# modal-labs/modal-client

Hardware: AMD Instinct MI355X
Metric: map_items_per_sec (higher is better)
Workload: dtype bf16; 1 GPU; model=Function.map fan-out (BASELINE config 3), global_batch=12500, seq_len=0, parallelism=map1, dynamic_batching=64, chunk_items=256, workers=8

## Files before the change

csrc/core.cpp:

```cpp

#include <pybind11/pybind11.h>
#include <pybind11/stl.h>

#include "lane.h"
#include "ring.h"

#include <algorithm>
#include <atomic>
#include <functional>
#include <thread>
#include <cerrno>
#include <cstdint>
#include <cstring>
#include <fcntl.h>
#include <stdexcept>
#include <string>
#include <sys/mman.h>
#include <sys/stat.h>
#include <unistd.h>
#include <vector>

namespace py = pybind11;

namespace {

using modal_amd::BellFile;
using modal_amd::Ring;
using modal_amd::RingHub;

constexpr uint64_t kGilReleaseBytes = 64 * 1024;

bool ring_push(Ring& ring, py::buffer buf) {
  py::buffer_info info = buf.request();
  const uint8_t* src = static_cast<const uint8_t*>(info.ptr);
  const uint64_t n = (uint64_t)info.size * (uint64_t)info.itemsize;
  uint8_t* dst = ring.reserve(n);
  if (!dst) return false;
  if (n >= kGilReleaseBytes) {
    py::gil_scoped_release release;
    std::memcpy(dst, src, n);
  } else {
    std::memcpy(dst, src, n);
  }
  ring.commit();
  return true;
}

py::list ring_pop_all(Ring& ring, size_t max_frames) {
  py::list out;
  ring.pop(
      [&](const uint8_t* ptr, size_t len) {
        out.append(py::bytes(reinterpret_cast<const char*>(ptr), len));
      },
      max_frames);
  return out;
}

py::list hub_drain(RingHub& hub) {
  py::list out;
  hub.drain([&](int slot, const uint8_t* ptr, size_t len) {
    out.append(py::make_tuple(slot, py::bytes(reinterpret_cast<const char*>(ptr), len)));
  });
  return out;
}

using modal_amd::Assignment;
using modal_amd::ChunkDone;
using modal_amd::ChunkLane;
using modal_amd::FrameKind;

py::str sv_str(std::string_view s) { return py::str(s.data(), s.size()); }

py::tuple done_tuple(const ChunkDone& d) {
  py::object cis = py::none();
  if (!d.cis_nil) {
    py::list items;
    for (int64_t v : d.cis) items.append(py::int_(v));
    cis = std::move(items);
  }
  return py::make_tuple(sv_str(d.token), sv_str(d.call_id), sv_str(d.chunk_id),
                        sv_str(d.function_id), py::int_(d.count),
                        py::bytes(d.data.data(), d.data.size()), cis);
}

py::list assignment_list(const std::vector<Assignment>& assignments) {
  py::list out;
  for (const auto& a : assignments) out.append(py::make_tuple(a.token, a.worker_slot));
  return out;
}

py::object parse_chunk_done_py(py::buffer buf) {
  py::buffer_info info = buf.request();
  ChunkDone done;
  FrameKind kind = modal_amd::parse_chunk_done(
      static_cast<const uint8_t*>(info.ptr), (size_t)info.size * (size_t)info.itemsize, &done);
  if (kind != FrameKind::kDoneClean) return py::none();
  return done_tuple(done);
}

int lane_submit(ChunkLane& lane, int fn_slot, const std::string& token, uint64_t count,
                py::buffer frame, bool front) {
  py::buffer_info info = frame.request();
  return lane.submit(fn_slot, token, count, static_cast<const uint8_t*>(info.ptr),
                     (size_t)info.size * (size_t)info.itemsize, front);
}

py::tuple lane_drain(ChunkLane& lane, RingHub& hub) {
  py::list completions, raw;
  std::vector<Assignment> assignments;
  lane.drain(
      hub,
      [&](int slot, const ChunkDone& done) {
        completions.append(py::make_tuple(slot, done_tuple(done)));
      },
      [&](int slot, const uint8_t* ptr, size_t len) {
        raw.append(py::make_tuple(slot, py::bytes(reinterpret_cast<const char*>(ptr), len)));
      },
      &assignments);
  return py::make_tuple(completions, raw, assignment_list(assignments));
}

py::bytes pack_payloads(const std::vector<py::bytes>& items) {
  uint64_t total = 0;
  std::vector<std::pair<const char*, size_t>> views;
  views.reserve(items.size());
  for (const auto& item : items) {
    char* ptr;
    Py_ssize_t n;
    if (PyBytes_AsStringAndSize(item.ptr(), &ptr, &n) != 0)
      throw std::runtime_error("pack_payloads: not bytes");
// ... 319 lines not shown
  }
  if (pid < 0) {
    if (cg_fd >= 0) ::close(cg_fd);
    throw std::runtime_error("clone3: " + std::string(strerror(errno)));
  }
  if (pid == 0) {
    ::setsid();
    if (stdin_fd >= 0) ::dup2(stdin_fd, 0);
    if (stdout_fd >= 0) ::dup2(stdout_fd, 1);
    if (stderr_fd >= 0) ::dup2(stderr_fd, 2);
    for (int fd = 3; fd < 1024; ++fd) ::close(fd);
    if (!cwd.empty() && ::chdir(cwd.c_str()) != 0) _exit(126);
    if (rlimit_as_mib > 0) {
      struct rlimit rl;
      rl.rlim_cur = rl.rlim_max = (rlim_t)rlimit_as_mib << 20;
      ::setrlimit(RLIMIT_AS, &rl);
    }
    ::execve(cargv[0], cargv.data(), cenv.data());
    _exit(127);
  }
  if (cg_fd >= 0) ::close(cg_fd);
  return (int64_t)pid;
}


PYBIND11_MODULE(_core, m) {
  m.doc() = "modal_amd native core: shm ring transport + batch framing";
  py::class_<BellFile, std::shared_ptr<BellFile>>(m, "BellFile")
      .def(py::init<const std::string&, bool>(), py::arg("path"), py::arg("create") = false);
  py::class_<Ring, std::shared_ptr<Ring>>(m, "ShmRing")
      .def(py::init<const std::string&, uint64_t, bool>(), py::arg("path"),
           py::arg("capacity") = (uint64_t)64 << 20, py::arg("create") = false)
      .def("push", &ring_push)
      .def("pop_all", &ring_pop_all, py::arg("max_frames") = 0)
      .def("pending_bytes", &Ring::pending_bytes)
      .def("capacity", &Ring::capacity)
      .def("too_large", &Ring::too_large)
      .def("bell_wakes", &Ring::bell_wakes)
      .def("set_shared_bell", &Ring::set_shared_bell);
  py::class_<RingHub>(m, "RingHub")
      .def(py::init<const std::string&, int>(), py::arg("bell_path") = "",
           py::arg("timeout_ms") = 20)
      .def("add_ring", &RingHub::add_ring)
      .def("remove_ring", &RingHub::remove_ring)
      .def("fd", &RingHub::fd)
      .def("drain", &hub_drain)
      .def("close", &RingHub::close)
      .def("stats", [](RingHub& hub) {
        py::dict d;
        d["notifies"] = hub.notifies();
        d["waits"] = hub.waits();
        d["drains"] = hub.drains();
        d["producer_wakes"] = hub.producer_wakes();
        d["rings"] = hub.ring_count();
        return d;
      });
  py::class_<ChunkLane>(m, "ChunkLane")
      .def(py::init<>())
      .def("add_worker", &ChunkLane::add_worker)
      .def("remove_worker", &ChunkLane::remove_worker)
      .def("set_eligible", &ChunkLane::set_eligible)
      .def("set_cap", &ChunkLane::set_cap, py::arg("fn_slot"), py::arg("items"),
           py::arg("min_chunks") = 1)
      .def("submit", &lane_submit, py::arg("fn_slot"), py::arg("token"), py::arg("count"),
           py::arg("frame"), py::arg("front") = false)
      .def("kick", [](ChunkLane& lane, int fn_slot) {
        std::vector<Assignment> out;
        lane.kick(fn_slot, &out);
        return assignment_list(out);
      })
      .def("complete", [](ChunkLane& lane, int worker_slot, const std::string& token) {
        std::vector<Assignment> out;
        lane.complete(worker_slot, token, &out);
        return assignment_list(out);
      })
      .def("cancel", &ChunkLane::cancel)
      .def("drop_queue", &ChunkLane::drop_queue)
      .def("drain", &lane_drain)
      .def("queued", &ChunkLane::queued)
      .def("inflight", &ChunkLane::inflight)
      .def("outstanding_items", &ChunkLane::outstanding_items)
      .def("pushed", &ChunkLane::pushed);
  m.def("parse_chunk_done", &parse_chunk_done_py);
  m.def("pack_payloads", &pack_payloads);
  m.def("malz_compress", &malz_compress, py::arg("data"), py::arg("min_gain") = 0.95);
  m.def("malz_decompress", &malz_decompress);
  m.def("unpack_payloads", &unpack_payloads);
  m.def("spawn_supervised", &spawn_supervised, py::arg("argv"), py::arg("cwd"),
        py::arg("env"), py::arg("cgroup_dir") = "", py::arg("rlimit_as_mib") = 0,
        py::arg("stdin_fd") = -1, py::arg("stdout_fd") = -1, py::arg("stderr_fd") = -1,
        "clone3(CLONE_INTO_CGROUP) + execve supervisor (atomic cgroup placement)");
}
```

csrc/lane.h:

```cpp

#pragma once

#include <algorithm>
#include <cstdint>
#include <cstring>
#include <deque>
#include <memory>
#include <string>
#include <string_view>
#include <unordered_map>
#include <unordered_set>
#include <utility>
#include <vector>

#include "ring.h"

namespace modal_amd {


struct MsgReader {
  const uint8_t* p;
  const uint8_t* end;

  bool need(size_t n) const { return (size_t)(end - p) >= n; }
// ... 198 lines not shown
        if (r.need(1) && *r.p == 0xc0) {
          r.p++;
          out->cis_nil = true;
          break;
        }
        uint64_t n;
        ok = r.read_array_header(&n) && n <= (uint64_t)(r.end - r.p);
        out->cis_nil = false;
        out->cis.clear();
        for (uint64_t k = 0; ok && k < n; k++) {
          int64_t v;
          ok = r.read_int(&v);
          if (ok) out->cis.push_back(v);
        }
        break;
      }
    }
    if (!ok) {
      r.p = value_at;
      if (!r.skip()) return FrameKind::kOther;
      clean = false;
      if (bit == T) return FrameKind::kOther;
      if (bit == TOKEN) has_token = false;
    }
  }
  if (r.p != r.end) return FrameKind::kOther;
  if (!is_done || !has_token) return FrameKind::kOther;
  out->token = token;
  if (clean && seen == 255) return FrameKind::kDoneClean;
  return FrameKind::kDoneOther;
}


struct Assignment {
  std::string token;
  int worker_slot;
};

class ChunkLane {
 public:
  void add_worker(int slot, std::shared_ptr<Ring> ring) {
    Worker& w = workers_[slot];
    w.ring = std::move(ring);
  }

  std::vector<std::string> remove_worker(int slot) {
    std::vector<std::string> tokens;
    auto it = workers_.find(slot);
    if (it == workers_.end()) return tokens;
    for (auto& entry : it->second.inflight) tokens.push_back(entry.first);
    workers_.erase(it);
    for (auto& fn : fns_) fn.second.eligible.erase(slot);
    return tokens;
  }

  void set_eligible(int fn_slot, int worker_slot, bool on) {
    Fn& fn = fns_[fn_slot];
    if (on && workers_.count(worker_slot)) fn.eligible.insert(worker_slot);
    else fn.eligible.erase(worker_slot);
  }

  void set_cap(int fn_slot, uint64_t items, uint32_t min_chunks) {
    Fn& fn = fns_[fn_slot];
    fn.cap_items = items;
    fn.min_chunks = min_chunks;
  }
// ... 6 lines not shown
      if (slot >= 0) return slot;
    }
    Queued q{token, count, std::string(reinterpret_cast<const char*>(frame), len)};
    if (front) fn.queue.push_front(std::move(q));
    else fn.queue.push_back(std::move(q));
    return -1;
  }

  void kick(int fn_slot, std::vector<Assignment>* out) {
    auto it = fns_.find(fn_slot);
    if (it == fns_.end()) return;
    Fn& fn = it->second;
    while (!fn.queue.empty()) {
      Queued& q = fn.queue.front();
      int slot = place(fn_slot, fn, q.token, q.count,
                       reinterpret_cast<const uint8_t*>(q.frame.data()), q.frame.size(),
                       fn.queue.size());
      if (slot < 0) break;
      out->push_back(Assignment{std::move(q.token), slot});
      fn.queue.pop_front();
    }
  }

  bool complete(int worker_slot, std::string_view token, std::vector<Assignment>* out) {
    auto wit = workers_.find(worker_slot);
    if (wit == workers_.end()) return false;
    Worker& w = wit->second;
    auto it = w.inflight.find(std::string(token));
    if (it == w.inflight.end()) return false;
    int fn_slot = it->second.fn_slot;
    Load& load = w.load[fn_slot];
    load.items -= std::min(load.items, it->second.count);
    if (load.chunks) load.chunks--;
    w.inflight.erase(it);
    kick(fn_slot, out);
    return true;
  }

  std::vector<std::string> cancel(const std::vector<std::string>& tokens) {
    std::unordered_set<std::string_view> drop(tokens.begin(), tokens.end());
    std::vector<std::string> dropped;
    for (auto& entry : fns_) {
      auto& q = entry.second.queue;
      auto keep = q.begin();
      for (auto it = q.begin(); it != q.end(); ++it) {
        if (drop.count(it->token)) {
          dropped.push_back(std::move(it->token));
        } else {
          if (keep != it) *keep = std::move(*it);
          ++keep;
        }
      }
      q.erase(keep, q.end());
    }
    return dropped;
  }

  std::vector<std::string> drop_queue(int fn_slot) {
    std::vector<std::string> tokens;
    auto it = fns_.find(fn_slot);
    if (it == fns_.end()) return tokens;
    for (auto& q : it->second.queue) tokens.push_back(std::move(q.token));
    it->second.queue.clear();
    return tokens;
  }

  template <typename OnClean, typename OnRaw>
  void drain(RingHub& hub, OnClean&& on_clean, OnRaw&& on_raw, std::vector<Assignment>* out) {
    ChunkDone done;
    hub.drain([&](int slot, const uint8_t* ptr, size_t len) {
      FrameKind kind = parse_chunk_done(ptr, len, &done);
      if (kind != FrameKind::kOther) complete(slot, done.token, out);
      if (kind == FrameKind::kDoneClean) on_clean(slot, done);
      else on_raw(slot, ptr, len);
    });
  }

  size_t queued(int fn_slot) const {
    auto it = fns_.find(fn_slot);
    return it == fns_.end() ? 0 : it->second.queue.size();
  }

  size_t inflight(int worker_slot) const {
    auto it = workers_.find(worker_slot);
    return it == workers_.end() ? 0 : it->second.inflight.size();
  }

  uint64_t outstanding_items(int fn_slot, int worker_slot) const {
    auto it = workers_.find(worker_slot);
    if (it == workers_.end()) return 0;
    auto lit = it->second.load.find(fn_slot);
    return lit == it->second.load.end() ? 0 : lit->second.items;
  }

  uint64_t pushed() const { return pushed_; }

 private:
  struct Queued {
    std::string token;
    uint64_t count;
    std::string frame;
  };
  struct Load {
    uint64_t items = 0;
    uint32_t chunks = 0;
  };
  struct Inflight {
    int fn_slot;
    uint64_t count;
  };
  struct Worker {
    std::shared_ptr<Ring> ring;
    std::unordered_map<int, Load> load;
    std::unordered_map<std::string, Inflight> inflight;
  };
  struct Fn {
    uint64_t cap_items = 256;
    uint32_t min_chunks = 1;
    std::deque<Queued> queue;
    std::unordered_set<int> eligible;
  };

  static bool has_credit(const Fn& fn, const Load& load, size_t backlog) {
    if (load.items < fn.cap_items) return true;
    return load.chunks < fn.min_chunks && backlog > fn.eligible.size();
  }

  int place(int fn_slot, Fn& fn, const std::string& token, uint64_t count,
            const uint8_t* frame, size_t len, size_t backlog) {
    std::vector<std::pair<uint64_t, int>> order;
    for (int slot : fn.eligible) {
      auto it = workers_.find(slot);
      if (it == workers_.end()) continue;
      const Load& load = it->second.load[fn_slot];
      if (has_credit(fn, load, backlog)) order.emplace_back(load.items, slot);
    }
    std::sort(order.begin(), order.end());
    for (auto& cand : order) {
      Worker& w = workers_[cand.second];
      if (w.ring->too_large(len) || !w.ring->push(frame, len)) continue;
      Load& load = w.load[fn_slot];
      load.items += count;
      load.chunks++;
      w.inflight[token] = Inflight{fn_slot, count};
      pushed_++;
      return cand.second;
    }
    return -1;
  }

  std::unordered_map<int, Worker> workers_;
  std::unordered_map<int, Fn> fns_;
  uint64_t pushed_ = 0;
};

}
```

csrc/ring.h:

```cpp

#pragma once

#include <atomic>
#include <cerrno>
#include <climits>
#include <cstdint>
#include <cstring>
#include <ctime>
#include <fcntl.h>
#include <linux/futex.h>
#include <memory>
#include <csignal>
#include <pthread.h>
#include <mutex>
#include <stdexcept>
#include <string>
#include <sys/eventfd.h>
#include <sys/mman.h>
#include <sys/stat.h>
#include <sys/syscall.h>
#include <thread>
#include <unistd.h>
#include <utility>
#include <vector>
// ... 92 lines not shown
      ::close(fd_);
      throw std::runtime_error("ShmRing: mmap failed");
    }
    base_ = static_cast<uint8_t*>(mem);
    header_ = reinterpret_cast<RingHeader*>(base_);
    data_ = base_ + sizeof(RingHeader);
    total_ = total;
    if (create) {
      header_->head.store(0, std::memory_order_relaxed);
      header_->tail.store(0, std::memory_order_relaxed);
      header_->capacity = capacity;
      header_->bell.seq.store(0, std::memory_order_relaxed);
      header_->bell.waiting.store(0, std::memory_order_relaxed);
      header_->bell.wakes.store(0, std::memory_order_relaxed);
      header_->magic = kMagic;
    } else if (header_->magic != kMagic || header_->capacity != capacity) {
      ::munmap(base_, total_);
      ::close(fd_);
      throw std::runtime_error("ShmRing: magic mismatch");
    }
    capacity_ = capacity;
  }

  ~Ring() {
    if (base_) ::munmap(base_, total_);
    if (fd_ >= 0) ::close(fd_);
  }

  Ring(const Ring&) = delete;
  Ring& operator=(const Ring&) = delete;

  bool too_large(uint64_t n) const { return n + 8 > capacity_ || n >= kSkip; }

  uint8_t* reserve(uint64_t n) {
    if (too_large(n)) throw std::runtime_error("frame larger than ring");
    uint64_t head = header_->head.load(std::memory_order_relaxed);
    uint64_t tail = header_->tail.load(std::memory_order_acquire);
    uint64_t pos = head % capacity_;
    uint64_t to_end = capacity_ - pos;
    uint64_t need = 4 + n;
    uint64_t skip = to_end < need ? to_end : 0;
    if (head + skip + need - tail > capacity_) return nullptr;
    if (skip) {
      if (to_end >= 4) {
        uint32_t sentinel = kSkip;
        std::memcpy(data_ + pos, &sentinel, 4);
      }
      pos = 0;
    }
    uint32_t len32 = (uint32_t)n;
    std::memcpy(data_ + pos, &len32, 4);
    pending_commit_ = head + skip + need;
    return data_ + pos + 4;
  }

  void commit() {
    header_->head.store(pending_commit_, std::memory_order_release);
    bell_ring(header_->bell);
    if (shared_bell_) bell_ring(*shared_bell_->bell());
  }

  bool push(const uint8_t* src, uint64_t n) {
    uint8_t* dst = reserve(n);
    if (!dst) return false;
    std::memcpy(dst, src, n);
    commit();
    return true;
  }

  template <typename F>
  size_t pop(F&& cb, size_t max_frames = 0) {
    uint64_t tail = header_->tail.load(std::memory_order_relaxed);
    uint64_t head = header_->head.load(std::memory_order_acquire);
    if (tail == head) return 0;
    size_t count = 0;
    while (tail < head) {
      uint64_t pos = tail % capacity_;
      uint64_t to_end = capacity_ - pos;
      if (to_end < 4) {
        tail += to_end;
        continue;
      }
      uint32_t len32;
      std::memcpy(&len32, data_ + pos, 4);
      if (len32 == kSkip) {
        tail += to_end;
        continue;
      }
      if ((uint64_t)len32 + 4 > to_end || tail + 4 + len32 > head) break;
      cb(static_cast<const uint8_t*>(data_ + pos + 4), (size_t)len32);
      tail += 4 + len32;
      if (max_frames && ++count >= max_frames) break;
    }
    header_->tail.store(tail, std::memory_order_release);
    return count;
  }

  bool has_pending() const {
    return header_->head.load(std::memory_order_acquire) !=
           header_->tail.load(std::memory_order_acquire);
  }

  uint64_t pending_bytes() const {
    return header_->head.load(std::memory_order_acquire) -
           header_->tail.load(std::memory_order_acquire);
  }

  uint64_t capacity() const { return capacity_; }
  Bell* bell() const { return &header_->bell; }
  uint32_t bell_wakes() const { return header_->bell.wakes.load(std::memory_order_relaxed); }

  void set_shared_bell(std::shared_ptr<BellFile> bell) { shared_bell_ = std::move(bell); }

 private:
  int fd_ = -1;
  uint8_t* base_ = nullptr;
  uint8_t* data_ = nullptr;
  RingHeader* header_ = nullptr;
  uint64_t capacity_ = 0;
  uint64_t total_ = 0;
  uint64_t pending_commit_ = 0;
  std::shared_ptr<BellFile> shared_bell_;
};

class RingHub {
 public:
  explicit RingHub(const std::string& bell_path = "", int timeout_ms = 20)
      : timeout_ms_(timeout_ms < 1 ? 1 : timeout_ms) {
    if (!bell_path.empty()) {
      bell_file_ = std::make_shared<BellFile>(bell_path, true);
      bell_ = bell_file_->bell();
    }
    efd_ = ::eventfd(0, EFD_NONBLOCK | EFD_CLOEXEC);
    if (efd_ < 0) throw std::runtime_error("RingHub: eventfd failed");
    thread_ = std::thread([this] { run(); });
  }

  ~RingHub() { close(); }
  RingHub(const RingHub&) = delete;
  RingHub& operator=(const RingHub&) = delete;

  void add_ring(int slot, std::shared_ptr<Ring> ring) {
    std::lock_guard<std::mutex> lock(mu_);
    for (auto& entry : rings_) {
      if (entry.first == slot) {
        entry.second = std::move(ring);
        return;
      }
    }
    if (!bell_) {
      bell_owner_ = ring;
      bell_ = ring->bell();
    }
    rings_.emplace_back(slot, std::move(ring));
// ... 119 lines not shown
```

modal_amd/runtime/worker.py:

```python

from __future__ import annotations

import asyncio
import contextvars
import inspect
import os
import sys
import time
import traceback
from concurrent.futures import ThreadPoolExecutor
from typing import Any, Optional

from .._serialization import (
    DataFormat,
    GeneratorDone,
    deserialize,
    deserialize_payload,
    serialize,
    serialize_data_format,
    set_client_context,
)
from ..scheduler.blobs import INLINE_LIMIT, BlobStore
from ..scheduler.calls import (
    GENERIC_STATUS_FAILURE,
    GENERIC_STATUS_INTERNAL_FAILURE,
    GENERIC_STATUS_SUCCESS,
    GENERIC_STATUS_TERMINATED,
    GENERIC_STATUS_TIMEOUT,
)
from ..exception import InputCancellation
from ..scheduler.transport import Connection
from .execution_context import _reset_current_context, _set_current_context

HEARTBEAT_INTERVAL = 15.0
OUTPUT_FLUSH_INTERVAL = 0.001
OUTPUT_BATCH_MAX = 512

_app_id_var: contextvars.ContextVar[str] = contextvars.ContextVar("modal_amd_app_id", default="")

import threading as _threading

_slot_tls = _threading.local()


def _slot_streams_enabled() -> bool:
    torch = sys.modules.get("torch")
    cuda = getattr(torch, "cuda", None) if torch is not None else None
    try:
        return (
            cuda is not None
            and os.environ.get("MODAL_AMD_SLOT_STREAMS", "0") not in ("0", "false")
            and cuda.is_initialized()
        )
    except AttributeError:
        return False


def _invoke_on_slot_stream(fn: Any, args: tuple, kwargs: dict) -> Any:
    torch = sys.modules.get("torch")
    cuda = getattr(torch, "cuda", None) if torch is not None else None
    try:
        if (
            cuda is None
            or os.environ.get("MODAL_AMD_SLOT_STREAMS", "0") in ("0", "false")
            or not cuda.is_initialized()
        ):
            return fn(*args, **kwargs)
    except AttributeError:
        return fn(*args, **kwargs)
    stream = getattr(_slot_tls, "stream", None)
    if stream is None:
        stream = torch.cuda.Stream()
        _slot_tls.stream = stream
    with torch.cuda.stream(stream):
        result = fn(*args, **kwargs)
# ... 707 lines not shown
            prefix = f"in-{call_id[3:]}-"
            plain_call = not _slot_streams_enabled()
            tok_c = _current_function_call_id.set(call_id)
            tok_a = _app_id_var.set(frt.app_id)
            self._register_sync_thread(msg["token"])
            try:
                for ci in range(start, end):
                    tok_i = _current_input_id.set(prefix + str(ci))
                    try:
                        if kw_common is None:
                            args, kwargs = pairs[ci]
                        else:
                            args, kwargs = pairs[ci], kw_common
                        if plain_call:
                            values[ci] = fn(*args, **kwargs)
                        else:
                            values[ci] = _invoke_on_slot_stream(fn, args, kwargs)
                    except InputCancellation:
                        raise
                    except BaseException as exc:
                        errors[ci] = (
                            self._serialize_exception(exc),
                            "".join(traceback.format_exception_only(type(exc), exc)).strip(),
                        )
                    finally:
                        _current_input_id.reset(tok_i)
            finally:
                self._unregister_sync_thread(msg["token"])
                _current_function_call_id.reset(tok_c)
                _app_id_var.reset(tok_a)

        from .execution_context import _current_function_call_id, _current_input_id

        try:
            fn0 = await loop.run_in_executor(self.executor, frt.load)
            if frt._service is not None:
                fn0 = frt.get_callable(msg.get("method", ""))
        except BaseException as exc:
            data = self._serialize_exception(exc)
            err = "".join(traceback.format_exception_only(type(exc), exc)).strip()
            for ci in range(count):
                errors[ci] = (data, err)
            fn0 = None

        app_tok = _app_id_var.set(frt.app_id)
        try:
            if fn0 is not None and frt.batch_max_size > 1:
                is_async = inspect.iscoroutinefunction(fn0)

                def _transpose(pairs: Any, kw_common: Any, idxs: range) -> tuple:
                    rows = [
                        (pairs[ci], kw_common) if kw_common is not None else pairs[ci]
                        for ci in idxs
                    ]
                    if kw_common is not None:
                        n_args = len(rows[0][0]) if rows else 0
                        arglists = [[row[0][i] for row in rows] for i in range(n_args)]
                        kwlists = {k: [v] * len(rows) for k, v in kw_common.items()}
                    else:
                        n_args = max((len(a) for a, _ in rows), default=0)
                        arglists = [
                            [a[i] if i < len(a) else None for a, _ in rows]
                            for i in range(n_args)
                        ]
                        keys: set = set()
                        for _, kw in rows:
                            keys.update(kw)
                        kwlists = {k: [kw.get(k) for _, kw in rows] for k in keys}
                    return tuple(arglists), kwlists

                def _store(idxs: range, results: Any) -> None:
                    if not isinstance(results, (list, tuple)) or len(results) != len(idxs):
                        raise ValueError(
                            f"Batched function {frt.name} must return a list of "
                            f"{len(idxs)} results, got {type(results).__name__}"
                        )
                    for ci, r in zip(idxs, results):
                        values[ci] = r

                try:
                    pairs, kw_common = await loop.run_in_executor(
                        self.executor, self._chunk_pairs, msg["chunk_id"]
                    )
                    bsz = frt.batch_max_size
                    async with frt.sem:
                        for start in range(0, count, bsz):
                            idxs = range(start, min(start + bsz, count))
                            try:
                                arglists, kwlists = _transpose(pairs, kw_common, idxs)
                                if is_async:
                                    results = await self._execute(frt, fn0, arglists, kwlists)
                                else:

                                    def _call_batch(
                                        arglists: tuple = arglists, kwlists: dict = kwlists
                                    ) -> Any:
                                        tok_c = _current_function_call_id.set(call_id)
                                        tok_a2 = _app_id_var.set(frt.app_id)
                                        try:
                                            return fn0(*arglists, **kwlists)
                                        finally:
                                            _current_function_call_id.reset(tok_c)
                                            _app_id_var.reset(tok_a2)

                                    results = await loop.run_in_executor(
                                        self.executor, _call_batch
                                    )
                                _store(idxs, results)
                            except (asyncio.CancelledError, InputCancellation):
                                raise
                            except BaseException as exc:
                                data = self._serialize_exception(exc)
                                err = "".join(
                                    traceback.format_exception_only(type(exc), exc)
                                ).strip()
                                for ci in idxs:
                                    errors[ci] = (data, err)
                except (asyncio.CancelledError, InputCancellation):
                    raise
                except BaseException as exc:
                    data = self._serialize_exception(exc)
                    err = "".join(traceback.format_exception_only(type(exc), exc)).strip()
                    for ci in range(count):
                        errors.setdefault(ci, (data, err))
            elif fn0 is not None and (
                inspect.iscoroutinefunction(fn0) or inspect.isasyncgenfunction(fn0)
            ):
                item = {"chunk": msg["chunk_id"], "ci": 0}
                for ci in range(count):
                    item["ci"] = ci
                    try:
                        args, kwargs = await loop.run_in_executor(
                            self.executor, self._resolve_item_args, dict(item)
                        )
                        values[ci] = await self._execute(frt, fn0, args, kwargs)
                    except BaseException as exc:
                        errors[ci] = (
                            self._serialize_exception(exc),
                            "".join(traceback.format_exception_only(type(exc), exc)).strip(),
                        )
            elif fn0 is not None:
                if count <= frt.max_concurrent:
                    n_ranges = count
                else:
                    n_ranges = min(frt.max_concurrent, max(1, count // 16))
                size = (count + n_ranges - 1) // n_ranges

                async def run_one(start: int, end: int) -> None:
                    async with frt.sem:
                        await loop.run_in_executor(self.executor, run_range, start, end)

                await asyncio.gather(
                    *(run_one(s, min(s + size, count)) for s in range(0, count, size))
                )
        except (asyncio.CancelledError, InputCancellation):
            return
        finally:
            _app_id_var.reset(app_tok)

        reply: dict[str, Any] = {
            "t": "chunk_done",
            "token": token,
            "call_id": call_id,
            "chunk_id": msg["chunk_id"],
            "function_id": frt.function_id,
            "count": count,
        }
        if errors:
            reply["exceptions"] = {str(ci): [d, r] for ci, (d, r) in errors.items()}
        if values:
            ordered_cis = sorted(values)
            from ._serialize_chunk import serialize_value_chunk

            def pack() -> tuple:
                return serialize_value_chunk([values[ci] for ci in ordered_cis])

            data, per_item = await loop.run_in_executor(self.executor, pack)
            if data is not None:
                reply["data"] = data
                reply["cis"] = None if len(ordered_cis) == count else ordered_cis
            else:
                reply["items"] = {str(ci): b for ci, b in zip(ordered_cis, per_item)}
        try:
            await self.conn.send(reply)
        except Exception:
            pass

    async def _run_frame_fast(self, frt: FunctionRuntime, items: list[dict]) -> None:
        loop = asyncio.get_running_loop()
        from .execution_context import _current_function_call_id, _current_input_id

        def run_all() -> Any:
            results: list[dict] = []
            try:
                fn = frt.get_callable(items[0].get("method", ""))
            except BaseException as exc:
                err = "".join(traceback.format_exception_only(type(exc), exc)).strip()
                data = self._serialize_exception(exc)
                return [
                    self._make_output(
                        item["token"], frt.function_id, GENERIC_STATUS_FAILURE, data,
                        DataFormat.PICKLE, err,
                    )
                    for item in items
                ]
            if inspect.iscoroutinefunction(fn) or inspect.isasyncgenfunction(fn) or inspect.isgeneratorfunction(fn):
                return None
            values: list = []
            value_tokens: list[str] = []
            for item in items:
                if item["token"] in self._abandoned:
                    self._abandoned.discard(item["token"])
                    continue
                call_id = item["token"].rsplit(":", 2)[0]
                tok_i = _current_input_id.set(item.get("input_id"))
                tok_c = _current_function_call_id.set(call_id)
                try:
                    args, kwargs = self._resolve_item_args(item)
                    values.append(fn(*args, **kwargs))
# ... 335 lines not shown
```

modal_amd/scheduler/transport.py:

```python

from __future__ import annotations

import asyncio
import os
import itertools
import struct
from collections import deque
from typing import Any, Awaitable, Callable, Optional

import msgpack

_LEN = struct.Struct("<I")

MAX_FRAME = 1 << 31

RING_MIN_FRAME = int(os.environ.get("MODAL_AMD_RING_MIN", 32 * 1024))
RING_CAPACITY = 64 << 20

try:
    from .. import _core
except ImportError:
    _core = None


# ... 17 lines not shown
    except (asyncio.IncompleteReadError, ConnectionResetError):
        return None
    (length,) = _LEN.unpack(header)
    if length > MAX_FRAME:
        raise ValueError(f"Frame too large: {length}")
    try:
        body = await reader.readexactly(length)
    except (asyncio.IncompleteReadError, ConnectionResetError):
        return None
    return msgpack.unpackb(body, raw=False, strict_map_key=False)


class Connection:

    def __init__(
        self,
        reader: asyncio.StreamReader,
        writer: asyncio.StreamWriter,
        handler: Callable[[dict], Awaitable[None]],
        rpc_target: Optional[Any] = None,
    ):
        self.reader = reader
        self.writer = writer
        self.handler = handler
        self.rpc_target = rpc_target
        self._rpc_seq = itertools.count(1)
        self._pending: dict[int, asyncio.Future] = {}
        self._send_lock = asyncio.Lock()
        self._closed = asyncio.Event()
        self._reader_task: Optional[asyncio.Task] = None
        self._loop: Optional[asyncio.AbstractEventLoop] = None
        self.ring_out: Any = None
        self.ring_in: Any = None
        self.ring_frames_sent = 0
        self.ring_frames_received = 0
        self._lane = False
        self._own_hub: Any = None
        self.sync_handler: Optional[Callable[[dict], bool]] = None
        self._inbox: deque = deque()
        self._lane_waiting = 0
        self._inbox_task: Optional[asyncio.Task] = None

    def attach_rings(self, out_path: Optional[str], in_path: Optional[str], create: bool) -> bool:
        if _core is None or not out_path or not in_path:
            return False
        try:
            self.ring_out = _core.ShmRing(out_path, RING_CAPACITY, create)
            self.ring_in = _core.ShmRing(in_path, RING_CAPACITY, create)
            return True
        except Exception:
            self.ring_out = None
            self.ring_in = None
            return False

    def enable_lane(self, shared_bell: Optional[str] = None, own_hub: bool = False) -> bool:
        if _core is None or self.ring_out is None or self.ring_in is None:
            return False
        try:
            if shared_bell:
                self.ring_out.set_shared_bell(_core.BellFile(shared_bell, False))
            if own_hub:
                hub = _core.RingHub("", 20)
                hub.add_ring(0, self.ring_in)
                asyncio.get_running_loop().add_reader(hub.fd(), self._on_own_hub_ready)
                self._own_hub = hub
        except Exception:
            self._drop_own_hub()
            return False
        self._lane = True
        return True

    def _on_own_hub_ready(self) -> None:
        hub = self._own_hub
        if hub is None:
# ... 12 lines not shown

    def on_ring_frame(self, body: bytes) -> None:
        self.ring_frames_received += 1
        msg = msgpack.unpackb(body, raw=False, strict_map_key=False)
        if self._inbox_task is None:
            if msg.get("t") in _RPC_REPLY_KINDS:
                self._on_rpc_reply(msg)
                return
            if self.sync_handler is not None and self.sync_handler(msg):
                return
            self._inbox_task = asyncio.get_running_loop().create_task(self._run_inbox())
        self._inbox.append(msg)

    async def _run_inbox(self) -> None:
        try:
            while self._inbox:
                msg = self._inbox.popleft()
                try:
                    await self._dispatch(msg)
                except asyncio.CancelledError:
                    raise
                except Exception:
                    pass
        finally:
            self._inbox_task = None
            if self._inbox and not self._closed.is_set():
                self._inbox_task = asyncio.get_running_loop().create_task(self._run_inbox())

    async def _send_lane(self, body: bytes) -> None:
        if self._closed.is_set():
            raise ConnectionError("connection closed")
        ring = self.ring_out
        if self._lane_waiting == 0 and ring.push(body):
            self.ring_frames_sent += 1
            return
        self._lane_waiting += 1
        try:
            async with self._send_lock:
                while not ring.push(body):
                    if self._closed.is_set():
                        raise ConnectionError("connection closed")
                    await asyncio.sleep(0.001)
                self.ring_frames_sent += 1
        finally:
            self._lane_waiting -= 1

    def start(self) -> None:
        self._loop = asyncio.get_running_loop()
        self._reader_task = self._loop.create_task(self._read_loop())

    @property
    def closed(self) -> bool:
        return self._closed.is_set()

    async def wait_closed(self) -> None:
        await self._closed.wait()

    async def send(self, msg: dict, via_socket: bool = False) -> None:
        body = msgpack.packb(msg, use_bin_type=True)
        if self._lane and not via_socket:
            await self._send_lane(body)
            return
        if self.ring_out is not None and len(body) >= RING_MIN_FRAME and not via_socket:
            pushed = self.ring_out.push(body)
            if pushed:
                self.ring_frames_sent += 1
                async with self._send_lock:
                    self.writer.write(pack({"t": "rb"}))
                    await self.writer.drain()
                return
        data = _LEN.pack(len(body)) + body
        async with self._send_lock:
            self.writer.write(data)
            await self.writer.drain()

    async def call(self, method: str, params: Any = None, timeout: Optional[float] = None) -> Any:
        running = asyncio.get_running_loop()
        if self._loop is not None and running is not self._loop:
            fut = asyncio.run_coroutine_threadsafe(self.call(method, params, timeout), self._loop)
            return await asyncio.wrap_future(fut)
        rpc_id = next(self._rpc_seq)
        fut: asyncio.Future = asyncio.get_running_loop().create_future()
        self._pending[rpc_id] = fut
        try:
            await self.send({"t": "rpc", "i": rpc_id, "m": method, "p": params})
            if timeout is not None:
                return await asyncio.wait_for(fut, timeout)
            return await fut
        finally:
            self._pending.pop(rpc_id, None)

    async def _dispatch(self, msg: dict) -> None:
        kind = msg.get("t")
        if kind == "rpc":
            asyncio.get_running_loop().create_task(self._serve_rpc(msg))
        elif kind in _RPC_REPLY_KINDS:
            self._on_rpc_reply(msg)
        else:
            await self.handler(msg)
# ... 82 lines not shown
```

modal_amd/scheduler/workerhost.py:

```python

from __future__ import annotations

import asyncio
import heapq
import os
import subprocess
import sys
import time
from collections import deque
from typing import TYPE_CHECKING, Any, Optional

import msgpack

from ..utils.ids import new_id
from .calls import (
    GENERIC_STATUS_INTERNAL_FAILURE,
    MAX_INTERNAL_FAILURE_COUNT,
    FunctionDef,
    InputRecord,
)
from .transport import Connection, _core, native_lane_enabled

_CPU_COUNT = os.cpu_count()

# ... 155 lines not shown
                "call_id": record.call_id,
                "chunk_id": group.chunk_id,
                "token": group.token,
                "count": group.count,
                "payload": chunk.get("data"),
                "method": group.method,
                "max_concurrent": fdef.max_concurrent_inputs,
            },
            use_bin_type=True,
        )
        if len(frame) > LANE_MAX_FRAME:
            return False
        fn_slot = self._lane_fn_slot(fdef)
        token = group.token
        self._lane_groups[token] = (record, group)
        slot = self._lane.submit(fn_slot, token, group.count, frame, front)
        if slot >= 0:
            self._lane_assigned(token, slot)
        else:
            self._lane_refresh_fns.add(fdef.function_id)
            self._dispatch_wake.set()
        return True

    def _lane_assigned(self, token: str, slot: int) -> None:
        entry = self._lane_groups.get(token)
        w = self._lane_workers.get(slot)
        if entry is None or w is None:
            return
        record, group = entry
        group.state = "inflight"
        group.worker_id = w.worker_id
        w.last_active = time.time()
        w.inflight[token] = ("g", record, group)
        w.conn.ring_frames_sent += 1
        fid = record.function_id
        w.outstanding[fid] = w.outstanding.get(fid, 0) + group.count

    def _lane_revoke(self, w: WorkerHandle) -> None:
        if self._lane is not None and w.hub_slot is not None:
            for fid in w.lane_fns:
                self._lane.set_eligible(self._lane_fn_slots[fid], w.hub_slot, False)
        w.lane_fns.clear()

    async def _lane_dispatch(self) -> None:
        lane = self._lane
        for fid in list(self._lane_refresh_fns):
            self._lane_refresh_fns.discard(fid)
            fn_slot = self._lane_fn_slots.get(fid)
            if lane is None or fn_slot is None:
                continue
            fdef = self.scheduler.functions.get(fid)
            if fdef is None:
                for token in lane.drop_queue(fn_slot):
                    self._lane_groups.pop(token, None)
                continue
            fn_slot = self._lane_fn_slot(fdef)
            await self.ensure_workers(fdef.needs_gpu)
            candidates = [
                w
                for w in self.workers.values()
                if w.alive and not w.draining and (w.has_gpu or not fdef.needs_gpu)
            ]
            candidates = self._apply_placement(fdef, candidates)
            chosen = {w.worker_id for w in candidates}
            for w in list(self._lane_workers.values()):
                if fid in w.lane_fns and w.worker_id not in chosen:
                    w.lane_fns.discard(fid)
# ... 876 lines not shown
```

Baseline: 1.707 million items/s.

## Run chunk jobs in one executor call and push chunk_done natively from the worker thread

Map-chunk execution on the worker becomes a single executor job that runs the function, serializes the results and encodes the chunk_done reply straight into the shared-memory ring in C++ with the GIL released. This removes event-loop round trips, Python msgpack packing and a copy per chunk. The ring gains a producer mutex so several threads can push safely, and its push counter now tracks frames sent. It also adds per-chunk turnaround timing (clock_gettime on placement and completion) and a stress test, which cost a little per chunk and add some complexity around cancellation.

```diff
diff --git a/csrc/core.cpp b/csrc/core.cpp
--- a/csrc/core.cpp
+++ b/csrc/core.cpp
@@ -34,16 +34,11 @@
   py::buffer_info info = buf.request();
   const uint8_t* src = static_cast<const uint8_t*>(info.ptr);
   const uint64_t n = (uint64_t)info.size * (uint64_t)info.itemsize;
-  uint8_t* dst = ring.reserve(n);
-  if (!dst) return false;
   if (n >= kGilReleaseBytes) {
     py::gil_scoped_release release;
-    std::memcpy(dst, src, n);
-  } else {
-    std::memcpy(dst, src, n);
-  }
-  ring.commit();
-  return true;
+    return ring.push(src, n);
+  }
+  return ring.push(src, n);
 }
 
 py::list ring_pop_all(Ring& ring, size_t max_frames) {
@@ -96,6 +91,65 @@
       static_cast<const uint8_t*>(info.ptr), (size_t)info.size * (size_t)info.itemsize, &done);
   if (kind != FrameKind::kDoneClean) return py::none();
   return done_tuple(done);
+}
+
+struct DoneFields {
+  std::string_view token, call_id, chunk_id, function_id, data;
+  uint64_t count;
+  size_t size;
+};
+
+std::string_view ascii_view(const py::str& s, const char* what) {
+  if (!PyUnicode_IS_ASCII(s.ptr()))
+    throw py::value_error(std::string("chunk_done: ") + what + " is not ASCII");
+  Py_ssize_t n = 0;
+  const char* ptr = PyUnicode_AsUTF8AndSize(s.ptr(), &n);
+  if (!ptr) throw py::error_already_set();
+  if ((uint64_t)n > 0xffffffffULL)
+    throw py::value_error(std::string("chunk_done: ") + what + " is too long");
+  return std::string_view(ptr, (size_t)n);
+}
+
+DoneFields done_fields(const py::str& token, const py::str& call_id, const py::str& chunk_id,
+                       const py::str& function_id, int64_t count,
+                       const py::buffer_info& data) {
+  if (count < 0) throw py::value_error("chunk_done: count is negative");
+  DoneFields f;
+  f.token = ascii_view(token, "token");
+  f.call_id = ascii_view(call_id, "call_id");
+  f.chunk_id = ascii_view(chunk_id, "chunk_id");
+  f.function_id = ascii_view(function_id, "function_id");
+  uint64_t n = (uint64_t)data.size * (uint64_t)data.itemsize;
+  if (n > 0xffffffffULL) throw py::value_error("chunk_done: data is too long");
+  f.data = std::string_view(static_cast<const char*>(data.ptr), (size_t)n);
+  f.count = (uint64_t)count;
+  f.size = modal_amd::chunk_done_size(f.token, f.call_id, f.chunk_id, f.function_id, f.count,
+                                      f.data.size());
+  return f;
+}
+
+py::bytes build_chunk_done(const py::str& token, const py::str& call_id,
+                           const py::str& chunk_id, const py::str& function_id,
+                           int64_t count, py::buffer data) {
+  py::buffer_info info = data.request();
+  DoneFields f = done_fields(token, call_id, chunk_id, function_id, count, info);
+  py::bytes out(nullptr, (ssize_t)f.size);
+  uint8_t* dst = reinterpret_cast<uint8_t*>(PyBytes_AsString(out.ptr()));
+  modal_amd::encode_chunk_done(dst, f.token, f.call_id, f.chunk_id, f.function_id, f.count,
+                               f.data);
+  return out;
+}
+
+bool ring_push_chunk_done(Ring& ring, const py::str& token, const py::str& call_id,
+                          const py::str& chunk_id, const py::str& function_id,
+                          int64_t count, py::buffer data) {
+  py::buffer_info info = data.request();
+  DoneFields f = done_fields(token, call_id, chunk_id, function_id, count, info);
+  py::gil_scoped_release release;
+  return ring.push_with(f.size, [&](uint8_t* dst) {
+    modal_amd::encode_chunk_done(dst, f.token, f.call_id, f.chunk_id, f.function_id, f.count,
+                                 f.data);
+  });
 }
 
 int lane_submit(ChunkLane& lane, int fn_slot, const std::string& token, uint64_t count,
@@ -481,6 +535,9 @@
       .def(py::init<const std::string&, uint64_t, bool>(), py::arg("path"),
            py::arg("capacity") = (uint64_t)64 << 20, py::arg("create") = false)
       .def("push", &ring_push)
+      .def("push_chunk_done", &ring_push_chunk_done, py::arg("token"), py::arg("call_id"),
+           py::arg("chunk_id"), py::arg("function_id"), py::arg("count"), py::arg("data"))
+      .def("pushed", &Ring::pushed)
       .def("pop_all", &ring_pop_all, py::arg("max_frames") = 0)
       .def("pending_bytes", &Ring::pending_bytes)
       .def("capacity", &Ring::capacity)
@@ -529,8 +586,18 @@
       .def("queued", &ChunkLane::queued)
       .def("inflight", &ChunkLane::inflight)
       .def("outstanding_items", &ChunkLane::outstanding_items)
-      .def("pushed", &ChunkLane::pushed);
+      .def("pushed", &ChunkLane::pushed)
+      .def("stats", [](ChunkLane& lane, int fn_slot, bool reset) {
+        ChunkLane::Turnaround t = lane.stats(fn_slot, reset);
+        py::dict d;
+        d["chunks"] = t.chunks;
+        d["sum_ns"] = t.sum_ns;
+        d["max_ns"] = t.max_ns;
+        return d;
+      }, py::arg("fn_slot"), py::arg("reset") = false);
   m.def("parse_chunk_done", &parse_chunk_done_py);
+  m.def("build_chunk_done", &build_chunk_done, py::arg("token"), py::arg("call_id"),
+        py::arg("chunk_id"), py::arg("function_id"), py::arg("count"), py::arg("data"));
   m.def("pack_payloads", &pack_payloads);
   m.def("malz_compress", &malz_compress, py::arg("data"), py::arg("min_gain") = 0.95);
   m.def("malz_decompress", &malz_decompress);
diff --git a/csrc/lane.h b/csrc/lane.h
--- a/csrc/lane.h
+++ b/csrc/lane.h
@@ -254,6 +254,87 @@
 }
 
 
+inline size_t mp_str_size(size_t n) {
+  return n + (n < 32 ? 1 : n < 256 ? 2 : n < 65536 ? 3 : 5);
+}
+inline size_t mp_bin_size(size_t n) { return n + (n < 256 ? 2 : n < 65536 ? 3 : 5); }
+inline size_t mp_uint_size(uint64_t v) {
+  return v < 128 ? 1 : v < 256 ? 2 : v < 65536 ? 3 : v <= 0xffffffffULL ? 5 : 9;
+}
+
+inline uint8_t* mp_put_be(uint8_t* p, uint64_t v, int n) {
+  for (int i = n - 1; i >= 0; i--) *p++ = (uint8_t)(v >> (8 * i));
+  return p;
+}
+inline uint8_t* mp_put_str(uint8_t* p, std::string_view s) {
+  size_t n = s.size();
+  if (n < 32) *p++ = (uint8_t)(0xa0 | n);
+  else if (n < 256) { *p++ = 0xd9; p = mp_put_be(p, n, 1); }
+  else if (n < 65536) { *p++ = 0xda; p = mp_put_be(p, n, 2); }
+  else { *p++ = 0xdb; p = mp_put_be(p, n, 4); }
+  if (n) std::memcpy(p, s.data(), n);
+  return p + n;
+}
+inline uint8_t* mp_put_bin(uint8_t* p, std::string_view s) {
+  size_t n = s.size();
+  if (n < 256) { *p++ = 0xc4; p = mp_put_be(p, n, 1); }
+  else if (n < 65536) { *p++ = 0xc5; p = mp_put_be(p, n, 2); }
+  else { *p++ = 0xc6; p = mp_put_be(p, n, 4); }
+  if (n) std::memcpy(p, s.data(), n);
+  return p + n;
+}
+inline uint8_t* mp_put_uint(uint8_t* p, uint64_t v) {
+  if (v < 128) { *p++ = (uint8_t)v; return p; }
+  if (v < 256) { *p++ = 0xcc; return mp_put_be(p, v, 1); }
+  if (v < 65536) { *p++ = 0xcd; return mp_put_be(p, v, 2); }
+  if (v <= 0xffffffffULL) { *p++ = 0xce; return mp_put_be(p, v, 4); }
+  *p++ = 0xcf;
+  return mp_put_be(p, v, 8);
+}
+
+constexpr size_t kChunkDoneFixed =
+    1 + 2 + 11 + 6 + 8 + 9 + 12 + 6 + 5 + 4 + 1;
+
+inline size_t chunk_done_size(std::string_view token, std::string_view call_id,
+                              std::string_view chunk_id, std::string_view function_id,
+                              uint64_t count, size_t data_len) {
+  return kChunkDoneFixed + mp_str_size(token.size()) + mp_str_size(call_id.size()) +
+         mp_str_size(chunk_id.size()) + mp_str_size(function_id.size()) +
+         mp_uint_size(count) + mp_bin_size(data_len);
+}
+
+inline uint8_t* encode_chunk_done(uint8_t* dst, std::string_view token,
+                                  std::string_view call_id, std::string_view chunk_id,
+                                  std::string_view function_id, uint64_t count,
+                                  std::string_view data) {
+  uint8_t* p = dst;
+  *p++ = 0x88;
+  p = mp_put_str(p, "t");
+  p = mp_put_str(p, "chunk_done");
+  p = mp_put_str(p, "token");
+  p = mp_put_str(p, token);
+  p = mp_put_str(p, "call_id");
+  p = mp_put_str(p, call_id);
+  p = mp_put_str(p, "chunk_id");
+  p = mp_put_str(p, chunk_id);
+  p = mp_put_str(p, "function_id");
+  p = mp_put_str(p, function_id);
+  p = mp_put_str(p, "count");
+  p = mp_put_uint(p, count);
+  p = mp_put_str(p, "data");
+  p = mp_put_bin(p, data);
+  p = mp_put_str(p, "cis");
+  *p++ = 0xc0;
+  return p;
+}
+
+
+inline uint64_t monotonic_ns() {
+  struct timespec ts;
+  ::clock_gettime(CLOCK_MONOTONIC, &ts);
+  return (uint64_t)ts.tv_sec * 1000000000ULL + (uint64_t)ts.tv_nsec;
+}
+
 struct Assignment {
   std::string token;
   int worker_slot;
@@ -326,6 +407,12 @@
     Load& load = w.load[fn_slot];
     load.items -= std::min(load.items, it->second.count);
     if (load.chunks) load.chunks--;
+    uint64_t now = monotonic_ns();
+    uint64_t took = now > it->second.placed_ns ? now - it->second.placed_ns : 0;
+    Turnaround& t = fns_[fn_slot].turnaround;
+    t.chunks++;
+    t.sum_ns += took;
+    t.max_ns = std::max(t.max_ns, took);
     w.inflight.erase(it);
     kick(fn_slot, out);
     return true;
@@ -389,6 +476,20 @@
 
   uint64_t pushed() const { return pushed_; }
 
+  struct Turnaround {
+    uint64_t chunks = 0;
+    uint64_t sum_ns = 0;
+    uint64_t max_ns = 0;
+  };
+
+  Turnaround stats(int fn_slot, bool reset = false) {
+    auto it = fns_.find(fn_slot);
+    if (it == fns_.end()) return Turnaround{};
+    Turnaround t = it->second.turnaround;
+    if (reset) it->second.turnaround = Turnaround{};
+    return t;
+  }
+
  private:
   struct Queued {
     std::string token;
@@ -402,6 +503,7 @@
   struct Inflight {
     int fn_slot;
     uint64_t count;
+    uint64_t placed_ns;
   };
   struct Worker {
     std::shared_ptr<Ring> ring;
@@ -413,6 +515,7 @@
     uint32_t min_chunks = 1;
     std::deque<Queued> queue;
     std::unordered_set<int> eligible;
+    Turnaround turnaround;
   };
 
   static bool has_credit(const Fn& fn, const Load& load, size_t backlog) {
@@ -436,7 +539,7 @@
       Load& load = w.load[fn_slot];
       load.items += count;
       load.chunks++;
-      w.inflight[token] = Inflight{fn_slot, count};
+      w.inflight[token] = Inflight{fn_slot, count, monotonic_ns()};
       pushed_++;
       return cand.second;
     }
diff --git a/csrc/ring.h b/csrc/ring.h
--- a/csrc/ring.h
+++ b/csrc/ring.h
@@ -148,6 +148,24 @@
 
   bool too_large(uint64_t n) const { return n + 8 > capacity_ || n >= kSkip; }
 
+  template <typename W>
+  bool push_with(uint64_t n, W&& writer) {
+    std::lock_guard<std::mutex> lock(producer_mu_);
+    uint8_t* dst = reserve(n);
+    if (!dst) return false;
+    writer(dst);
+    commit();
+    pushed_.fetch_add(1, std::memory_order_relaxed);
+    return true;
+  }
+
+  bool push(const uint8_t* src, uint64_t n) {
+    return push_with(n, [&](uint8_t* dst) { std::memcpy(dst, src, n); });
+  }
+
+  uint64_t pushed() const { return pushed_.load(std::memory_order_relaxed); }
+
+ private:
   uint8_t* reserve(uint64_t n) {
     if (too_large(n)) throw std::runtime_error("frame larger than ring");
     uint64_t head = header_->head.load(std::memory_order_relaxed);
@@ -176,14 +194,7 @@
     if (shared_bell_) bell_ring(*shared_bell_->bell());
   }
 
-  bool push(const uint8_t* src, uint64_t n) {
-    uint8_t* dst = reserve(n);
-    if (!dst) return false;
-    std::memcpy(dst, src, n);
-    commit();
-    return true;
-  }
-
+ public:
   template <typename F>
   size_t pop(F&& cb, size_t max_frames = 0) {
     uint64_t tail = header_->tail.load(std::memory_order_relaxed);
@@ -236,6 +247,8 @@
   uint64_t capacity_ = 0;
   uint64_t total_ = 0;
   uint64_t pending_commit_ = 0;
+  std::mutex producer_mu_;
+  std::atomic<uint64_t> pushed_{0};
   std::shared_ptr<BellFile> shared_bell_;
 };
 
diff --git a/csrc/ring_producers_stress.cpp b/csrc/ring_producers_stress.cpp
--- /dev/null
+++ b/csrc/ring_producers_stress.cpp
@@ -0,0 +1,139 @@
+
+#include <atomic>
+#include <cstdio>
+#include <cstdlib>
+#include <string>
+#include <thread>
+#include <vector>
+
+#include "lane.h"
+#include "ring.h"
+
+using namespace modal_amd;
+
+namespace {
+
+constexpr int kProducers = 3;
+constexpr int kFrames = 20000;
+constexpr uint64_t kRingBytes = 64 * 1024;
+constexpr size_t kPlainHeader = 10;
+
+#define CHECK(cond)                                                      \
+  do {                                                                   \
+    if (!(cond)) {                                                       \
+      std::fprintf(stderr, "CHECK failed: %s (line %d)\n", #cond, __LINE__); \
+      std::abort();                                                      \
+    }                                                                    \
+  } while (0)
+
+size_t body_len(int producer, int seq) {
+  return 1024 + (size_t)(((uint32_t)seq * 2654435761u + (uint32_t)producer * 40503u) % 3072);
+}
+
+void fill(uint8_t* dst, size_t n, int producer, int seq) {
+  uint32_t x = (uint32_t)seq * 747796405u + (uint32_t)producer + 1u;
+  for (size_t i = 0; i < n; i++) {
+    x = x * 1664525u + 1013904223u;
+    dst[i] = (uint8_t)(x >> 24);
+  }
+}
+
+uint32_t checksum(const uint8_t* p, size_t n) {
+  uint32_t h = 2166136261u;
+  for (size_t i = 0; i < n; i++) h = (h ^ p[i]) * 16777619u;
+  return h;
+}
+
+void produce(Ring& ring, int producer) {
+  std::vector<uint8_t> body;
+  for (int seq = 0; seq < kFrames; seq++) {
+    size_t n = body_len(producer, seq);
+    body.resize(n);
+    fill(body.data(), n, producer, seq);
+    uint32_t sum = checksum(body.data(), n);
+    if (seq % 4 == 3) {
+      std::string token = "p" + std::to_string(producer) + ":" + std::to_string(seq);
+      std::string_view data(reinterpret_cast<const char*>(body.data()), n);
+      size_t size = chunk_done_size(token, "fc-stress", token.substr(1), "fu-stress", sum, n);
+      auto write = [&](uint8_t* dst) {
+        uint8_t* end = encode_chunk_done(dst, token, "fc-stress", token.substr(1), "fu-stress",
+                                         sum, data);
+        CHECK((size_t)(end - dst) == size);
+      };
+      while (!ring.push_with(size, write)) std::this_thread::yield();
+    } else {
+      auto write = [&](uint8_t* dst) {
+        dst[0] = 'P';
+        dst[1] = (uint8_t)producer;
+        uint32_t seq32 = (uint32_t)seq;
+        std::memcpy(dst + 2, &seq32, 4);
+        std::memcpy(dst + 6, &sum, 4);
+        std::memcpy(dst + kPlainHeader, body.data(), n);
+      };
+      while (!ring.push_with(kPlainHeader + n, write)) std::this_thread::yield();
+    }
+  }
+}
+
+}
+
+int main() {
+  char dir_template[] = "/tmp/ring-producers-XXXXXX";
+  CHECK(::mkdtemp(dir_template) != nullptr);
+  std::string dir = dir_template;
+  {
+    Ring tx(dir + "/ring", kRingBytes, true);
+    Ring rx(dir + "/ring", 0, false);
+
+    std::vector<std::thread> producers;
+    for (int p = 0; p < kProducers; p++) producers.emplace_back([&tx, p] { produce(tx, p); });
+
+    std::vector<int> next_seq(kProducers, 0);
+    int total = 0, encoded = 0;
+    ChunkDone done;
+    while (total < kProducers * kFrames) {
+      size_t got = rx.pop([&](const uint8_t* ptr, size_t len) {
+        int producer, seq;
+        uint32_t sum;
+        const uint8_t* body;
+        size_t n;
+        CHECK(len > kPlainHeader);
+        if (ptr[0] == 'P') {
+          producer = ptr[1];
+          uint32_t seq32;
+          std::memcpy(&seq32, ptr + 2, 4);
+          std::memcpy(&sum, ptr + 6, 4);
+          seq = (int)seq32;
+          body = ptr + kPlainHeader;
+          n = len - kPlainHeader;
+        } else {
+          CHECK(parse_chunk_done(ptr, len, &done) == FrameKind::kDoneClean);
+          CHECK(done.cis_nil && done.call_id == "fc-stress" && done.function_id == "fu-stress");
+          CHECK(done.token.size() > 3 && done.token[0] == 'p' && done.token[2] == ':');
+          CHECK(done.chunk_id == done.token.substr(1));
+          producer = done.token[1] - '0';
+          seq = std::atoi(std::string(done.token.substr(3)).c_str());
+          sum = (uint32_t)done.count;
+          body = reinterpret_cast<const uint8_t*>(done.data.data());
+          n = done.data.size();
+          CHECK(seq % 4 == 3);
+          encoded++;
+        }
+        CHECK(producer >= 0 && producer < kProducers);
+        CHECK(seq == next_seq[producer]);
+        next_seq[producer]++;
+        CHECK(n == body_len(producer, seq));
+        CHECK(checksum(body, n) == sum);
+        total++;
+      });
+      if (!got) std::this_thread::yield();
+    }
+    for (auto& t : producers) t.join();
+    CHECK(!rx.has_pending());
+    CHECK(tx.pushed() == (uint64_t)kProducers * kFrames);
+    CHECK(encoded == kProducers * (kFrames / 4));
+    std::printf("ring_producers_stress ok: %d frames, %d encoded natively\n", total, encoded);
+  }
+  std::string cmd = "rm -rf " + dir;
+  return std::system(cmd.c_str()) == 0 ? 0 : 1;
+}
diff --git a/modal_amd/runtime/worker.py b/modal_amd/runtime/worker.py
--- a/modal_amd/runtime/worker.py
+++ b/modal_amd/runtime/worker.py
@@ -41,6 +41,22 @@
 import threading as _threading
 
 _slot_tls = _threading.local()
+
+
+def _chunk_job_enabled() -> bool:
+    return os.environ.get("MODAL_AMD_CHUNK_JOB", "1").lower() not in ("0", "false", "no")
+
+
+class _ChunkJob:
+
+    __slots__ = ("lock", "cancelled")
+
+    def __init__(self) -> None:
+        self.lock = _threading.Lock()
+        self.cancelled = False
+
+
+_JOB_CANCELLED = object()
 
 
 def _slot_streams_enabled() -> bool:
@@ -814,8 +830,13 @@
 
         from .execution_context import _current_function_call_id, _current_input_id
 
+        chunk_job = frt.batch_max_size > 1 and _chunk_job_enabled()
+        job_reply: Any = None
         try:
-            fn0 = await loop.run_in_executor(self.executor, frt.load)
+            if chunk_job and frt._loaded:
+                fn0 = frt.load()
+            else:
+                fn0 = await loop.run_in_executor(self.executor, frt.load)
             if frt._service is not None:
                 fn0 = frt.get_callable(msg.get("method", ""))
         except BaseException as exc:
@@ -860,51 +881,114 @@
                     for ci, r in zip(idxs, results):
                         values[ci] = r
 
-                try:
-                    pairs, kw_common = await loop.run_in_executor(
-                        self.executor, self._chunk_pairs, msg["chunk_id"]
-                    )
-                    bsz = frt.batch_max_size
-                    async with frt.sem:
-                        for start in range(0, count, bsz):
-                            idxs = range(start, min(start + bsz, count))
+                if chunk_job and not is_async:
+                    state = _ChunkJob()
+
+                    def _run_job() -> Any:
+                        tok_c = _current_function_call_id.set(call_id)
+                        tok_a2 = _app_id_var.set(frt.app_id)
+                        self._register_sync_thread(token)
+                        try:
                             try:
-                                arglists, kwlists = _transpose(pairs, kw_common, idxs)
-                                if is_async:
-                                    results = await self._execute(frt, fn0, arglists, kwlists)
-                                else:
-
-                                    def _call_batch(
-                                        arglists: tuple = arglists, kwlists: dict = kwlists
-                                    ) -> Any:
-                                        tok_c = _current_function_call_id.set(call_id)
-                                        tok_a2 = _app_id_var.set(frt.app_id)
-                                        try:
-                                            return fn0(*arglists, **kwlists)
-                                        finally:
-                                            _current_function_call_id.reset(tok_c)
-                                            _app_id_var.reset(tok_a2)
-
-                                    results = await loop.run_in_executor(
-                                        self.executor, _call_batch
-                                    )
-                                _store(idxs, results)
-                            except (asyncio.CancelledError, InputCancellation):
+                                pairs, kw_common = self._chunk_pairs(msg["chunk_id"])
+                                bsz = frt.batch_max_size
+                                for start in range(0, count, bsz):
+                                    if state.cancelled:
+                                        return _JOB_CANCELLED
+                                    idxs = range(start, min(start + bsz, count))
+                                    try:
+                                        arglists, kwlists = _transpose(pairs, kw_common, idxs)
+                                        _store(idxs, fn0(*arglists, **kwlists))
+                                    except InputCancellation:
+                                        raise
+                                    except BaseException as exc:
+                                        data = self._serialize_exception(exc)
+                                        err = "".join(
+                                            traceback.format_exception_only(type(exc), exc)
+                                        ).strip()
+                                        for ci in idxs:
+                                            errors[ci] = (data, err)
+                            except InputCancellation:
                                 raise
                             except BaseException as exc:
                                 data = self._serialize_exception(exc)
                                 err = "".join(
                                     traceback.format_exception_only(type(exc), exc)
                                 ).strip()
-                                for ci in idxs:
-                                    errors[ci] = (data, err)
-                except (asyncio.CancelledError, InputCancellation):
-                    raise
-                except BaseException as exc:
-                    data = self._serialize_exception(exc)
-                    err = "".join(traceback.format_exception_only(type(exc), exc)).strip()
-                    for ci in range(count):
-                        errors.setdefault(ci, (data, err))
+                                for ci in range(count):
+                                    errors.setdefault(ci, (data, err))
+                            reply = self._chunk_reply(frt, msg, values, errors)
+                            clean = (
+                                not errors
+                                and len(values) == count
+                                and reply.get("data") is not None
+                            )
+                            with state.lock:
+                                if state.cancelled:
+                                    return _JOB_CANCELLED
+                                if clean and self._push_chunk_done(reply):
+                                    return None
+                            return reply
+                        finally:
+                            self._unregister_sync_thread(token)
+                            _current_function_call_id.reset(tok_c)
+                            _app_id_var.reset(tok_a2)
+
+                    try:
+                        async with frt.sem:
+                            job_reply = await loop.run_in_executor(self.executor, _run_job)
+                    except (asyncio.CancelledError, InputCancellation):
+                        with state.lock:
+                            state.cancelled = True
+                        raise
+                    if job_reply is None or job_reply is _JOB_CANCELLED:
+                        return
+                else:
+                    try:
+                        pairs, kw_common = await loop.run_in_executor(
+                            self.executor, self._chunk_pairs, msg["chunk_id"]
+                        )
+                        bsz = frt.batch_max_size
+                        async with frt.sem:
+                            for start in range(0, count, bsz):
+                                idxs = range(start, min(start + bsz, count))
+                                try:
+                                    arglists, kwlists = _transpose(pairs, kw_common, idxs)
+                                    if is_async:
+                                        results = await self._execute(frt, fn0, arglists, kwlists)
+                                    else:
+
+                                        def _call_batch(
+                                            arglists: tuple = arglists, kwlists: dict = kwlists
+                                        ) -> Any:
+                                            tok_c = _current_function_call_id.set(call_id)
+                                            tok_a2 = _app_id_var.set(frt.app_id)
+                                            try:
+                                                return fn0(*arglists, **kwlists)
+                                            finally:
+                                                _current_function_call_id.reset(tok_c)
+                                                _app_id_var.reset(tok_a2)
+
+                                        results = await loop.run_in_executor(
+                                            self.executor, _call_batch
+                                        )
+                                    _store(idxs, results)
+                                except (asyncio.CancelledError, InputCancellation):
+                                    raise
+                                except BaseException as exc:
+                                    data = self._serialize_exception(exc)
+                                    err = "".join(
+                                        traceback.format_exception_only(type(exc), exc)
+                                    ).strip()
+                                    for ci in idxs:
+                                        errors[ci] = (data, err)
+                    except (asyncio.CancelledError, InputCancellation):
+                        raise
+                    except BaseException as exc:
+                        data = self._serialize_exception(exc)
+                        err = "".join(traceback.format_exception_only(type(exc), exc)).strip()
+                        for ci in range(count):
+                            errors.setdefault(ci, (data, err))
             elif fn0 is not None and (
                 inspect.iscoroutinefunction(fn0) or inspect.isasyncgenfunction(fn0)
             ):
@@ -940,10 +1024,27 @@
         finally:
             _app_id_var.reset(app_tok)
 
+        if job_reply is not None:
+            reply = job_reply
+        elif values:
+            reply = await loop.run_in_executor(
+                self.executor, self._chunk_reply, frt, msg, values, errors
+            )
+        else:
+            reply = self._chunk_reply(frt, msg, values, errors)
+        try:
+            await self.conn.send(reply)
+        except Exception:
+            pass
+
+    def _chunk_reply(self, frt: FunctionRuntime, msg: dict, values: dict, errors: dict) -> dict:
+        from ._serialize_chunk import serialize_value_chunk
+
+        count = msg["count"]
         reply: dict[str, Any] = {
             "t": "chunk_done",
-            "token": token,
-            "call_id": call_id,
+            "token": msg["token"],
+            "call_id": msg["call_id"],
             "chunk_id": msg["chunk_id"],
             "function_id": frt.function_id,
             "count": count,
@@ -952,21 +1053,28 @@
             reply["exceptions"] = {str(ci): [d, r] for ci, (d, r) in errors.items()}
         if values:
             ordered_cis = sorted(values)
-            from ._serialize_chunk import serialize_value_chunk
-
-            def pack() -> tuple:
-                return serialize_value_chunk([values[ci] for ci in ordered_cis])
-
-            data, per_item = await loop.run_in_executor(self.executor, pack)
+            data, per_item = serialize_value_chunk([values[ci] for ci in ordered_cis])
             if data is not None:
                 reply["data"] = data
                 reply["cis"] = None if len(ordered_cis) == count else ordered_cis
             else:
                 reply["items"] = {str(ci): b for ci, b in zip(ordered_cis, per_item)}
+        return reply
+
+    def _push_chunk_done(self, reply: dict) -> bool:
+        conn = self.conn
+        ring = conn.ring_out
+        if ring is None or not conn._lane or conn._lane_waiting or conn.closed:
+            return False
         try:
-            await self.conn.send(reply)
+            return bool(
+                ring.push_chunk_done(
+                    reply["token"], reply["call_id"], reply["chunk_id"],
+                    reply["function_id"], reply["count"], reply["data"],
+                )
+            )
         except Exception:
-            pass
+            return False
 
     async def _run_frame_fast(self, frt: FunctionRuntime, items: list[dict]) -> None:
         loop = asyncio.get_running_loop()
diff --git a/modal_amd/scheduler/transport.py b/modal_amd/scheduler/transport.py
--- a/modal_amd/scheduler/transport.py
+++ b/modal_amd/scheduler/transport.py
@@ -73,7 +73,6 @@
         self._loop: Optional[asyncio.AbstractEventLoop] = None
         self.ring_out: Any = None
         self.ring_in: Any = None
-        self.ring_frames_sent = 0
         self.ring_frames_received = 0
         self._lane = False
         self._own_hub: Any = None
@@ -81,6 +80,11 @@
         self._inbox: deque = deque()
         self._lane_waiting = 0
         self._inbox_task: Optional[asyncio.Task] = None
+
+    @property
+    def ring_frames_sent(self) -> int:
+        ring = self.ring_out
+        return ring.pushed() if ring is not None else 0
 
     def attach_rings(self, out_path: Optional[str], in_path: Optional[str], create: bool) -> bool:
         if _core is None or not out_path or not in_path:
@@ -159,7 +163,6 @@
             raise ConnectionError("connection closed")
         ring = self.ring_out
         if self._lane_waiting == 0 and ring.push(body):
-            self.ring_frames_sent += 1
             return
         self._lane_waiting += 1
         try:
@@ -168,7 +171,6 @@
                     if self._closed.is_set():
                         raise ConnectionError("connection closed")
                     await asyncio.sleep(0.001)
-                self.ring_frames_sent += 1
         finally:
             self._lane_waiting -= 1
 
@@ -191,7 +193,6 @@
         if self.ring_out is not None and len(body) >= RING_MIN_FRAME and not via_socket:
             pushed = self.ring_out.push(body)
             if pushed:
-                self.ring_frames_sent += 1
                 async with self._send_lock:
                     self.writer.write(pack({"t": "rb"}))
                     await self.writer.drain()
diff --git a/modal_amd/scheduler/workerhost.py b/modal_amd/scheduler/workerhost.py
--- a/modal_amd/scheduler/workerhost.py
+++ b/modal_amd/scheduler/workerhost.py
@@ -211,7 +211,6 @@
         group.worker_id = w.worker_id
         w.last_active = time.time()
         w.inflight[token] = ("g", record, group)
-        w.conn.ring_frames_sent += 1
         fid = record.function_id
         w.outstanding[fid] = w.outstanding.get(fid, 0) + group.count
 
```

Measured after the change: 1.698 million items/s. Within noise of the previous version (-0.5%).
